# mlysy/rodeo

Hardware: AMD Instinct MI355X
Metric: ODE steps/sec x batch (trajectory-steps/s), FitzHugh-Nagumo q=3, 4000 steps, solve_mv (higher is better)
Workload: dtype f64

## Files before the change

### rodeo_amd/csrc/solve_paths.hpp

```cpp
#pragma once
#include <stdint.h>
#include <stddef.h>
#include <type_traits>
#include <utility>
#include "common.hpp"
#include "rhs.hpp"
#include "solve_args.hpp"

namespace rk {

struct DenseItgArgs;
struct SimLogpost;
struct DaltonObs;

int check_cfg(const rk_solve_cfg* c, const rk_solve_in* in);
int make_args(const rk_solve_cfg* c, const rk_solve_in* in, const rk_solve_out* out, SolveArgs& a);
int begin_solve(rk_handle h);
int small_backward_pass(rk_handle h, const rk_solve_cfg* c, const SolveArgs& a, int mode);

bool dense_supported(const rk_solve_cfg* c, int mode);
int dense_check(const rk_solve_cfg* c, const rk_solve_in* in, int mode);
int dense_solve(rk_handle h, const rk_solve_cfg* c, const rk_solve_in* in, const rk_solve_out* out, int mode);
size_t dense_ws_bytes(const rk_solve_cfg* c, int mode);

enum JitKind : int {
    JIT_FWD = 0,
    JIT_FWD_STORE_PRED = 1,
    JIT_ITG = 2,
    JIT_TILE3 = 3,
    JIT_TILE4 = 4,
    JIT_TILEN = 5,
    JIT_SQRT = 6,
    JIT_FWD_M = 7,
    JIT_FWD_M_STORE_PRED = 8,
    JIT_DENSE_ITG = 9,
    JIT_ITG_M = 10,
    JIT_DALTON = 11,
    JIT_DALTON_STORE = 12,
    JIT_DALTON_TILE3 = 13,
    JIT_DALTON_TILE3_STORE = 14,
};
bool is_user_rhs(int rhs_id);
bool user_tile_available(const rk_solve_cfg* c, JitKind tile);
int user_forward_tile(rk_handle h, const rk_solve_cfg* c, const SolveArgs& a, double* tiles, JitKind tile);
int user_forward(rk_handle h, const rk_solve_cfg* c, const SolveArgs& a);
int user_forward_sqrt(rk_handle h, const rk_solve_cfg* c, const SolveArgs& a);
int user_rhs_check(const rk_solve_cfg* c);
int user_dalton(rk_handle h, const rk_solve_cfg* c, const SolveArgs& a, const DaltonObs& o, int n_bobs, bool store,
                bool tile, double* out);
int user_interrogate(rk_handle h, const rk_solve_cfg* c, const SolveArgs& a, double t, int step, const double* mp,
                     const double* vp, double* wm, double* mm_, double* vm);
bool user_dense_wanted(const rk_solve_cfg* c);
int user_dense_interrogate(rk_handle h, const rk_solve_cfg* c, const DenseItgArgs& a);

int sqrt_solve(rk_handle h, const rk_solve_cfg* c, const SolveArgs& a, int mode, double* ws, size_t ws_bytes);
size_t sqrt_ws_doubles(const rk_solve_cfg* c, int mode);
size_t fenrir_sqrt_item_doubles(int p);
int fenrir_sqrt_launch(rk_handle h, const rk_solve_cfg* c, const SolveArgs& a, const double* obs, const double* obs_w,
                       const double* obs_v, const int32_t* obs_ind, int n_obs, int n_bobs, double* logdens, double* states);

bool tile3_supported(const rk_solve_cfg* c, int mode);
int tile3_solve(rk_handle h, const rk_solve_cfg* c, const SolveArgs& a, double* tiles, int mode, const SimLogpost* lp = nullptr);
int tile3_backward(rk_handle h, const SolveArgs& a, double* tiles, int mode, const SimLogpost* lp = nullptr);
bool tile3_sim_logpost_supported(const rk_solve_cfg* c, int n_obs);
int tile3_solve_sim_logpost(rk_handle h, const rk_solve_cfg* c, const SolveArgs& a, double* tiles, const double* obs,
                            const int32_t* obs_ind, int n_obs, double noise_sd, const double* upars, int n_prior, double prior_sd,
                            double* logpost);
int tile3_fenrir_backward(rk_handle h, const SolveArgs& a, const double* tiles, const double* obs, const double* obs_w,
                          const double* obs_v, const int32_t* obs_ind, int n_obs, double* logdens);
bool tile4_supported(const rk_solve_cfg* c, int mode);
int tile4_solve(rk_handle h, const rk_solve_cfg* c, const SolveArgs& a, double* tiles, int mode);
size_t tile4_doubles(const rk_solve_cfg* c);
bool tilen_supported(const rk_solve_cfg* c, int mode);
int tilen_solve(rk_handle h, const rk_solve_cfg* c, const SolveArgs& a, double* tiles, double* ws, size_t ws_bytes, int mode);
size_t tilen_tile_doubles(const rk_solve_cfg* c);
size_t tilen_ws_doubles(const rk_solve_cfg* c, int mode);

enum class SolvePath { Dense, Sqrt, Tile3, Tile4, TileN, Small };

inline SolvePath solve_path(const rk_solve_cfg* c, int mode) {
    if (dense_supported(c, mode)) return SolvePath::Dense;
    if (tile4_supported(c, mode)) return SolvePath::Tile4;
    if (tile3_supported(c, mode)) return SolvePath::Tile3;
    if (tilen_supported(c, mode)) return SolvePath::TileN;
    return c->kalman_type == RK_KALMAN_SQRT ? SolvePath::Sqrt : SolvePath::Small;
}

inline int path_layout(SolvePath p, const rk_solve_cfg* c) {
    switch (p) {
        case SolvePath::Dense: return RK_LAYOUT_TRAJ_MAJOR;
        case SolvePath::Tile3: return RK_LAYOUT_TILE3;
        case SolvePath::Tile4: return RK_LAYOUT_TILE4;
        case SolvePath::TileN: return c->n_bstate == 4 ? RK_LAYOUT_TILE4 : RK_LAYOUT_TILEP;
        default: return RK_LAYOUT_BATCH_MINOR;
    }
}

template <int Lo, int Hi, class F>
bool dispatch_int(int v, F&& f) {
    if constexpr (Lo > Hi) {
        return false;
    } else {
        if (v == Lo) {
            f(std::integral_constant<int, Lo>{});
            return true;
        }
        return dispatch_int<Lo + 1, Hi>(v, std::forward<F>(f));
    }
}

template <class F>
bool with_builtin_rhs(int rhs_id, F&& f) {
    switch (rhs_id) {
        case RK_RHS_FITZHUGH_NAGUMO: f(FitzHughNagumo{}); return true;
        case RK_RHS_LORENZ63: f(Lorenz63{}); return true;
        case RK_RHS_HIGHER_ORDER: f(HigherOrder{}); return true;
    }
    return false;
}

}
```

### rodeo_amd/csrc/solve_tile3.hip

```cpp
#include <cstdlib>
#include "common.hpp"
#include "kalman_small.hpp"
#include "mfma_tile.hpp"
#include "philox.hpp"
#include "rhs.hpp"
#include "solve_args.hpp"
#include "solve_paths.hpp"
#include "solve_tile3_kernels.hpp"

namespace rk {

constexpr int CHUNK = 16;
constexpr int ITEM_BYTES = 3 * 128;
constexpr int BUF_BYTES = CHUNK * 4 * ITEM_BYTES;
constexpr int ZONE_BYTES = 64 * TILE_DOUBLES * 8;

__device__ __forceinline__ int lds_byte(int s, int g, int which, int idx) {
    const int item = s * 4 + g;
    return item * ITEM_BYTES + which * 128 + (tile_slot(s, g, idx) << 3);
}

__device__ __forceinline__ void tile3_gain_producers(const SolveArgs& a, const double* __restrict__ tiles, int D, int tw, int wave,
                                                     int lane, int n_tiles, size_t tstride, int n_chunks, char* lds_raw,
                                                     char* zones) {
    constexpr int P = 3;
    const int p = wave - 1;
    const int s = lane >> 2, g = lane & 3;
    int tau = tw * 4 + g;
    if (tau >= n_tiles) tau = n_tiles - 1;
    const int b = tau / D, blk = tau - b * D;
    double Q[P][P], R[P][P];
    load_block_consts<P>(a, blk, b, Q, R);
    int woff[12];
#pragma unroll
    for (int i = 0; i < 3; ++i)
#pragma unroll
        for (int j = 0; j < 4; ++j) woff[i * 4 + j] = lds_byte(s, g, 0, i * 4 + j);
    char* const zone = zones + p * ZONE_BYTES;
    const unsigned zone_lds = __builtin_amdgcn_readfirstlane(lds_addr(zone));
    int frow[6], fcol[6];
#pragma unroll
    for (int i = 0; i < 6; ++i) { const int j = 64 * i + lane; frow[i] = j / 24; fcol[i] = (j % 24) * 16; }
    const char* const wave_tiles = (const char*)(tiles + (size_t)tw * 4 * TILE_DOUBLES);
    auto fetch = [&](int ch) {
        const int n_hi = a.N - 1 - ch * CHUNK;
#pragma unroll
        for (int i = 0; i < 6; ++i) {
            const int n = n_hi - frow[i];
            lds_dma16(wave_tiles + (size_t)(n < 1 ? 1 : n) * tstride * 8 + fcol[i], zone_lds + 1024 * i);
        }
    };
    lds_dma_wait_all();
    if (p < n_chunks) fetch(p);
    double mf[P], Sf[P][P], mp[P], Sp[P][P], A[P][P], X[P][P], rpiv[P];
    for (int t = -3; t < n_chunks; ++t) {
        const int ch1 = t + 3, ch2 = t + 2, ch3 = t + 1;
        if (ch1 % 3 == p) {
            if (ch1 < n_chunks) {
                lds_dma_wait_all();
                double buf[TILE_DOUBLES];
#pragma unroll
                for (int k = 0; k < 6; ++k) {
                    const double2 v = *(const double2*)(zone + 96 * lane + 16 * k);
                    buf[2 * k] = v.x; buf[2 * k + 1] = v.y;
                }
                lds_reads_done();
                if (ch1 + 3 < n_chunks) fetch(ch1 + 3);
#pragma unroll
                for (int i = 0; i < P; ++i) {
#pragma unroll
                    for (int j = 0; j < P; ++j) Sf[i][j] = buf[i * 4 + j];
                    mf[i] = buf[i * 4 + 3];
                }
                predict_block<P>(Q, R, mf, Sf, mp, Sp);
            }
        } else if (ch2 >= 0 && ch2 % 3 == p) {
            if (ch2 < n_chunks) {
                double T[P][P];
                mm_nt<P, P, P>(Sf, Q, T);
#pragma unroll
                for (int i = 0; i < P; ++i)
#pragma unroll
                    for (int j = 0; j < P; ++j) { A[i][j] = Sp[i][j]; X[i][j] = T[j][i]; }
                lu_factor_fwd<P, P>(A, X, rpiv);
            }
        } else if (ch3 >= 0) {
            if (ch3 < n_chunks) {
                lu_back<P, P>(A, X, rpiv);
                const int n = a.N - 1 - ch3 * CHUNK - s;
                if (n >= 1) {
                    char* o = lds_raw + (ch3 & 1) * BUF_BYTES;
#pragma unroll
                    for (int i = 0; i < P; ++i) {
#pragma unroll
                        for (int j = 0; j < P; ++j) {
                            *(double*)(o + woff[i * 4 + j]) = Sp[i][j];
                            *(double*)(o + woff[i * 4 + j] + 128) = X[i][j];
                            *(double*)(o + woff[i * 4 + j] + 256) = Sf[i][j];
                        }
                        *(double*)(o + woff[i * 4 + 3]) = mp[i];
                        *(double*)(o + woff[i * 4 + 3] + 256) = mf[i];
                    }
                }
            }
        }
        lds_barrier();   
    }
}

__global__ void __launch_bounds__(256) bwd_mv_tile3_kernel(SolveArgs a, double* __restrict__ tiles, int D) {
    __shared__ __attribute__((aligned(16))) char lds_all[2 * BUF_BYTES];
    __shared__ __attribute__((aligned(16))) char zones[3 * ZONE_BYTES];
    const int wave = threadIdx.x >> 6, lane = threadIdx.x & 63;
    const int n_tiles = a.B * D;
    const size_t tstride = (size_t)n_tiles * TILE_DOUBLES;
    const int n_chunks = (a.N - 1 + CHUNK - 1) / CHUNK;

    for (int i = threadIdx.x; i < 2 * 64 * 3 * 16; i += 256) {
        const int idx = i & 15, which = (i >> 4) % 3, item = ((i >> 4) / 3) & 63, buf = i / (64 * 3 * 16);
        const double v = (idx == 15) ? 1.0 : 0.0;
        *(double*)(lds_all + buf * BUF_BYTES + lds_byte(item >> 2, item & 3, which, idx)) = v;
    }
    __syncthreads();

    const int tw = blockIdx.x;
    char* const lds_raw = lds_all;
    double* const dump = tiles + (size_t)(a.N + 1) * tstride + (size_t)tw * 64;
    const int role = wave;

    if (role >= 1) {
        tile3_gain_producers(a, tiles, D, tw, role, lane, n_tiles, tstride, n_chunks, lds_raw, zones);
    } else {
        const TileCoord tc = tile_coord<1>(tw, lane, n_tiles);
        __builtin_amdgcn_s_setprio(3);
        const int r = tc.r, g = tc.g, c = tc.c, idx = r * 4 + c;
        const bool st = tc.valid && r < 3;
        double* base = st ? tiles + (size_t)tc.tau * TILE_DOUBLES + idx : dump + lane;
        const size_t ostride = st ? tstride : 0;
        int roff[4];
#pragma unroll
        for (int k = 0; k < 4; ++k) roff[k] = lds_byte(k, g, 0, idx) - k * 4 * ITEM_BYTES;
        double Ms = st ? base[(size_t)a.N * ostride] : ((r == 3 && c == 3) ? 1.0 : 0.0);
        const char* const wave_rows = (const char*)(tiles + (size_t)tw * 4 * TILE_DOUBLES);
        const size_t row_bytes = tstride * sizeof(double);
        const unsigned bvoff = st ? (unsigned)((g * TILE_DOUBLES + idx) * sizeof(double)) : 0x80000000u;
        const bool buffer_ok = (CHUNK - 1) * row_bytes + 384 < 0x7fffffffull;
        const int chunk_span = (int)((CHUNK - 1) * row_bytes + 384);
        lds_barrier();
        lds_barrier();
        lds_barrier();
        for (int t = 0; t < n_chunks; ++t) {
            const char* in = lds_raw + (t & 1) * BUF_BYTES;
            const int n_hi = a.N - 1 - t * CHUNK;
            const int cnt = __builtin_amdgcn_readfirstlane(n_hi >= CHUNK ? CHUNK : n_hi);
            double* o = base + (size_t)n_hi * ostride;
            {
                if (cnt == CHUNK && buffer_ok) {
                    constexpr int LOOKAHEAD = 4;
                    double Mp[CHUNK], Gt[CHUNK], Mf[CHUNK];
                    auto load = [&](int s) {
                        const char* q = in + roff[s & 3] + s * 4 * ITEM_BYTES;
                        Mp[s] = *(const double*)(q);
                        Gt[s] = *(const double*)(q + 128);
                        Mf[s] = *(const double*)(q + 256);
                    };
#pragma unroll
                    for (int s = 0; s < LOOKAHEAD; ++s) load(s);
                    const __amdgpu_buffer_rsrc_t rsrc = __builtin_amdgcn_make_buffer_rsrc(
                        (void*)(wave_rows + (size_t)(n_hi - (CHUNK - 1)) * row_bytes), 0, chunk_span, 0x00020000);
                    double Dm = Ms - Mp[0];
#pragma unroll
                    for (int s = 0; s < CHUNK; ++s) {
                        if (s + LOOKAHEAD < CHUNK) load(s + LOOKAHEAD);
                        __builtin_amdgcn_sched_barrier(0);
                        const double V1 = MF(Dm, Gt[s], 0.0);
                        Ms = MF(V1, Gt[s], Mf[s]);
                        if (s + 1 < CHUNK) Dm = Ms - Mp[s + 1];
                        u32x2 bits;
                        __builtin_memcpy(&bits, &Ms, 8);
                        __builtin_amdgcn_raw_buffer_store_b64(bits, rsrc, (int)bvoff, (int)((CHUNK - 1 - s) * row_bytes), 0);
                        __builtin_amdgcn_sched_barrier(0);
                    }
                } else {
                    for (int s = 0; s < cnt; ++s) {
                        const char* q = in + lds_byte(s, g, 0, idx);
                        const double Mp = *(const double*)(q), Gt = *(const double*)(q + 128), Mf = *(const double*)(q + 256);
                        const double V1 = MF(Ms - Mp, Gt, 0.0);
                        Ms = MF(V1, Gt, Mf);
                        o[0] = Ms;
                        o -= ostride;
                    }
                }
            }
            lds_barrier();   
        }
    }
}

struct FenrirObs {
    const double *obs, *obs_w, *obs_v;
    const int32_t* obs_ind;
    int n_obs;
    double* logdens;
};

__global__ void __launch_bounds__(256) fenrir_bwd_tile3_kernel(SolveArgs a, const double* __restrict__ tiles, int D, FenrirObs ob) {
    __shared__ __attribute__((aligned(16))) char lds_all[2 * BUF_BYTES];
    __shared__ __attribute__((aligned(16))) char zones[3 * ZONE_BYTES];
    const int wave = threadIdx.x >> 6, lane = threadIdx.x & 63;
    const int n_tiles = a.B * D;
    const size_t tstride = (size_t)n_tiles * TILE_DOUBLES;
    const int n_chunks = (a.N - 1 + CHUNK - 1) / CHUNK;

    for (int i = threadIdx.x; i < 2 * 64 * 3 * 16; i += 256) {
        const int idx = i & 15, which = (i >> 4) % 3, item = ((i >> 4) / 3) & 63, buf = i / (64 * 3 * 16);
        const double v = (idx == 15) ? 1.0 : 0.0;
        *(double*)(lds_all + buf * BUF_BYTES + lds_byte(item >> 2, item & 3, which, idx)) = v;
    }
    __syncthreads();

    const int tw = blockIdx.x;
    char* const lds_raw = lds_all;

    if (wave >= 1) {
        tile3_gain_producers(a, tiles, D, tw, wave, lane, n_tiles, tstride, n_chunks, lds_raw, zones);
    } else {
        __builtin_amdgcn_s_setprio(3);
        const int r = lane >> 4, g = (lane >> 2) & 3, c = lane & 3, idx = r * 4 + c;
        const int tau_raw = tw * 4 + g;
        const bool valid = tau_raw < n_tiles;
        const int tau = valid ? tau_raw : n_tiles - 1;
        const int b = tau / D, blk = tau - b * D;
        const bool in_tile = valid && r < 3;
        const double e3 = (r == 3 && c == 3) ? 1.0 : 0.0, I4 = r == c ? 1.0 : 0.0;
        const double* const my = tiles + (size_t)tau * TILE_DOUBLES + idx;
        int roff[4];
#pragma unroll
        for (int k = 0; k < 4; ++k) roff[k] = lds_byte(k, g, 0, idx) - k * 4 * ITEM_BYTES;
        double Ms = in_tile ? my[(size_t)a.N * tstride] : e3;
        double acc = 0.0;
        int i = ob.n_obs - 1;
        int next = i >= 0 ? ob.obs_ind[i] : -1;
        auto observe = [&]() {
            const double xw = valid ? (r < 3 ? ob.obs_w[((size_t)i * D + blk) * 3 + r] : -ob.obs[(size_t)i * D + blk]) : 0.0;
            const double Om = valid ? ob.obs_v[(size_t)i * D + blk] : 1.0;
            double MsT = MF(Ms, I4, 0.0);
            MsT = r == 3 ? 0.0 : MsT;
            const double WS = MF(xw, Ms, 0.0);
            const double Z = MF(MsT, xw, 0.0);
            const double w = MF(Z, xw, 0.0) + Om;
            const double z = -quad_bcast3(WS);
            if (fabs(w) > 1e-8) acc += -0.5 * (z * z / w + log(w)) - 0.5 * 1.83787706640934548356;
            const double K = Z / w;
            Ms = fma(-K, WS, Ms);
            --i;
            next = i >= 0 ? ob.obs_ind[i] : -1;
        };
        if (next >= a.N) observe();
        __syncthreads();
        __syncthreads();
        __syncthreads();
        for (int t = 0; t < n_chunks; ++t) {
            const char* in = lds_raw + (t & 1) * BUF_BYTES;
            const int n_hi = a.N - 1 - t * CHUNK;
            const int cnt = __builtin_amdgcn_readfirstlane(n_hi >= CHUNK ? CHUNK : n_hi);
            const bool has_obs = next > n_hi - cnt;
            if (cnt == CHUNK && !has_obs) {
                constexpr int LOOKAHEAD = 4;
                double Mp[CHUNK], Gt[CHUNK], Mf[CHUNK];
                auto load = [&](int s) {
                    const char* q = in + roff[s & 3] + s * 4 * ITEM_BYTES;
                    Mp[s] = *(const double*)(q);
                    Gt[s] = *(const double*)(q + 128);
                    Mf[s] = *(const double*)(q + 256);
                };
#pragma unroll
                for (int s = 0; s < LOOKAHEAD; ++s) load(s);
                double Dm = Ms - Mp[0];
#pragma unroll
                for (int s = 0; s < CHUNK; ++s) {
                    if (s + LOOKAHEAD < CHUNK) load(s + LOOKAHEAD);
                    __builtin_amdgcn_sched_barrier(0);
                    const double V1 = MF(Dm, Gt[s], 0.0);
                    Ms = MF(V1, Gt[s], Mf[s]);
                    if (s + 1 < CHUNK) Dm = Ms - Mp[s + 1];
                    __builtin_amdgcn_sched_barrier(0);
                }
            } else {
                for (int s = 0; s < cnt; ++s) {
                    const char* q = in + lds_byte(s, g, 0, idx);
                    const double Mp = *(const double*)(q), Gt = *(const double*)(q + 128), Mf = *(const double*)(q + 256);
                    const double V1 = MF(Ms - Mp, Gt, 0.0);
                    Ms = MF(V1, Gt, Mf);
                    if (next == n_hi - s) observe();
                }
            }
            __syncthreads();
        }
        if (next == 0) {
            Ms = in_tile ? my[0] : e3;
            observe();
        }
        if (valid && r == 0 && c == 0) atomicAdd(&ob.logdens[b], acc);
    }
}

constexpr int SIM_ITEM = 256;
constexpr int SIM_BUF = CHUNK * 4 * SIM_ITEM;

__device__ __forceinline__ int sim_tile_byte(int s, int g, int idx) {
    const int item = s * 4 + g;
    return item * SIM_ITEM + (tile_slot(s, g, idx) << 3);
}
__device__ __forceinline__ int sim_vec_byte(int s, int g, int which, int rr) {
    const int item = s * 4 + g;
    return item * SIM_ITEM + 128 + (vec_slot(s, g, which, rr) << 3);
}

struct SimLogpost {
    const double* obs;
    const int32_t* obs_ind;
    int n_obs;
    double noise_sd;
    const double* upars;
    int n_prior;
    double prior_sd;
    double* logpost;
};
constexpr int LP_MAX_OBS = 512, LP_MAX_VALS = 1024;

template <bool LP>
__global__ void __launch_bounds__(256, 2) bwd_sim_tile3_kernel(SolveArgs a, double* __restrict__ tiles, int D, SimLogpost lp) {
    constexpr int P = 3;
    __shared__ double lp_obs[LP ? LP_MAX_VALS : 1];
    __shared__ int lp_ind[LP ? LP_MAX_OBS : 1];
    if constexpr (LP) {
        for (int i = threadIdx.x; i < lp.n_obs * D; i += 256) lp_obs[i] = lp.obs[i];
        for (int i = threadIdx.x; i < lp.n_obs; i += 256) { const int ni = lp.obs_ind[i]; lp_ind[i] = ni < 0 ? 0 : (ni > a.N ? a.N : ni); }
    }
    __shared__ __attribute__((aligned(16))) char lds_all[2 * SIM_BUF];
    __shared__ __attribute__((aligned(16))) char zones[3 * ZONE_BYTES];
    constexpr int QR_STRIDE = 2 * 9 + 2;
    __shared__ __attribute__((aligned(16))) double qr[4 * QR_STRIDE];
    const int wave = threadIdx.x >> 6, lane = threadIdx.x & 63;
    const int n_tiles = a.B * D;
    const size_t tstride = (size_t)n_tiles * TILE_DOUBLES;
    const int n_chunks = (a.N + CHUNK - 1) / CHUNK;
// ... 104 lines not shown
                    z[2] = 0.125 + 1e-3 * n; z3 = 0.0;
#else
                    normal_pair(a.seed, traj, (uint32_t)(n < 1 ? 1 : n), (uint32_t)blk, PURPOSE_SMOOTH, 1u, z[2], z3);
#endif
                }
            } else if (ch3 >= 0) {
                if (ch3 < n_chunks) {
                    const int n = a.N - ch3 * CHUNK - s;
                    double GT[P][P], Ssim[P][P], L[P][P], G[P][P];
                    lu_back<P, P>(A, X, rpiv);
                    const bool term = n == a.N;
#pragma unroll
                    for (int i = 0; i < P; ++i)
#pragma unroll
                        for (int j = 0; j < P; ++j) G[i][j] = term ? 0.0 : X[j][i];
                    mm_nt<P, P, P>(G, T, GT);
#pragma unroll
                    for (int i = 0; i < P; ++i)
#pragma unroll
                        for (int j = 0; j < P; ++j) Ssim[i][j] = Sf[i][j] - GT[i][j];
#ifdef RK_T3_ABLATE_SIMPSD
#pragma unroll
                    for (int i = 0; i < P; ++i)
#pragma unroll
                        for (int j = 0; j < P; ++j) L[i][j] = Ssim[i][j];
#else
                    psd_factor<P>(Ssim, L);
#endif
                    if (n >= 1) {
                        char* o = lds_raw + (ch3 & 1) * SIM_BUF;
#pragma unroll
                        for (int i = 0; i < P; ++i) {
                            double w = mf[i];
#pragma unroll
                            for (int k = 0; k <= i; ++k) w = fma(L[i][k], z[k], w);
#pragma unroll
                            for (int j = 0; j < P; ++j) *(double*)(o + woff[i * 3 + j]) = G[j][i];
                            *(double*)(o + voff[i]) = term ? 0.0 : mp[i];
                            *(double*)(o + voff1[i]) = w;
                        }
                    }
                }
            }
            lds_barrier();
        }
    } else {
        const TileCoord tc = tile_coord<1>(tw, lane, n_tiles);
        const int r = tc.r, g = tc.g, c = tc.c, idx = r * 4 + c;
        const int b = tc.tau / D, blk = tc.tau - b * D;
        const bool st = tc.valid && r < 3 && c == 0 && a.x != nullptr;
        const size_t xstride = (size_t)D * P * a.B;
        double* bx = st ? a.x + ((size_t)blk * P + r) * a.B + b : dump + lane;
        const double LOG_SQRT_2PI = 0.91893853320467274178;
        const double lsd = LP ? log(lp.noise_sd) : 0.0;
        int io = LP ? lp.n_obs - 1 : -1;
        double acc = 0.0;
        auto next_index = [&]() { return io >= 0 ? __builtin_amdgcn_readfirstlane(lp_ind[io]) : -1; };
        auto observe = [&](double xv) {
            const double zz = (lp_obs[io * D + blk] - xv) / lp.noise_sd;
            acc += -0.5 * zz * zz - lsd - LOG_SQRT_2PI;
            --io;
        };
        const size_t sx = st ? xstride : 0;
        const bool xbuf_ok = (size_t)CHUNK * xstride * sizeof(double) < 0x7fffffffull;
        const int xvo = st && xbuf_ok ? (int)((((size_t)blk * P + r) * a.B + b) * sizeof(double)) : (int)0x80000000;
        int roff[4], rvec[4], rvec1[4];
#pragma unroll
        for (int k = 0; k < 4; ++k) {
            roff[k] = sim_tile_byte(k, g, idx) - k * 4 * SIM_ITEM;
            rvec[k] = sim_vec_byte(k, g, 0, r) - k * 4 * SIM_ITEM;
            rvec1[k] = sim_vec_byte(k, g, 1, r) - k * 4 * SIM_ITEM;
        }
        double x = 0.0;
        lds_barrier();
        int next_n = LP ? next_index() : -1;
        lds_barrier();
        lds_barrier();
        lds_barrier();
        for (int t = 0; t < n_chunks; ++t) {
            const char* in = lds_raw + (t & 1) * SIM_BUF;
            const int n_hi = a.N - t * CHUNK;
            const int cnt = __builtin_amdgcn_readfirstlane(n_hi >= CHUNK ? CHUNK : n_hi);
            double* o = bx + (size_t)n_hi * sx;
            auto step = [&](const char* q, const char* qv, const char* qw) {
                const double Gt = *(const double*)(q), mp = *(const double*)(qv), mfw = *(const double*)(qw);
                x = MF(Gt, x - mp, mfw);
                o[0] = x;
                o -= sx;
            };
            int n_cur = n_hi;
            if (cnt == CHUNK && xbuf_ok) {
                const __amdgpu_buffer_rsrc_t rsrc = __builtin_amdgcn_make_buffer_rsrc(
                    (void*)(a.x + (size_t)(n_hi - (CHUNK - 1)) * xstride), 0, (int)(CHUNK * xstride * sizeof(double)), 0x00020000);
                double xs[LP ? CHUNK : 1];
#pragma unroll
                for (int s = 0; s < CHUNK; ++s) {
                    const double Gt = *(const double*)(in + roff[s & 3] + s * 4 * SIM_ITEM);
                    const double mp = *(const double*)(in + rvec[s & 3] + s * 4 * SIM_ITEM);
                    const double mfw = *(const double*)(in + rvec1[s & 3] + s * 4 * SIM_ITEM);
                    x = MF(Gt, x - mp, mfw);
                    u32x2 bits;
                    __builtin_memcpy(&bits, &x, 8);
                    __builtin_amdgcn_raw_buffer_store_b64(bits, rsrc, xvo, (int)((CHUNK - 1 - s) * xstride * sizeof(double)), 0);
                    if constexpr (LP) xs[s] = x;
                }
                if constexpr (LP) {
                    if (next_n > n_hi - CHUNK) {
#pragma unroll
                        for (int s = 0; s < CHUNK; ++s)
                            while (n_hi - s == next_n) { observe(xs[s]); next_n = next_index(); }
                    }
                }
            } else if (cnt == CHUNK) {
#pragma unroll
                for (int s = 0; s < CHUNK; ++s) {
                    step(in + roff[s & 3] + s * 4 * SIM_ITEM, in + rvec[s & 3] + s * 4 * SIM_ITEM, in + rvec1[s & 3] + s * 4 * SIM_ITEM);
                    if constexpr (LP) {
                        while (n_cur == next_n) { observe(x); next_n = next_index(); }
                    }
                    --n_cur;
                }
            } else {
                for (int s = 0; s < cnt; ++s) {
                    step(in + sim_tile_byte(s, g, idx), in + sim_vec_byte(s, g, 0, r), in + sim_vec_byte(s, g, 1, r));
                    if constexpr (LP) {
                        while (n_cur == next_n) { observe(x); next_n = next_index(); }
                    }
                    --n_cur;
                }
            }
            lds_barrier();
        }
        const double x_init = tiles[(size_t)tc.tau * TILE_DOUBLES + r * 4 + 3];
        if (st) bx[0] = x_init;
        if constexpr (LP) {
            while (next_n == 0) { observe(x_init); next_n = next_index(); }
            if (D >= 2) acc += __shfl_xor(acc, 4, 64);
            if (D >= 4) acc += __shfl_xor(acc, 8, 64);
            if (tc.valid && r == 0 && c == 0 && blk == 0) {
                if (lp.upars) {
                    const double lps = log(lp.prior_sd);
                    for (int k = 0; k < lp.n_prior; ++k) {
                        const double zz = lp.upars[(size_t)k * a.B + b] / lp.prior_sd;
                        acc += -0.5 * zz * zz - lps - LOG_SQRT_2PI;
                    }
                }
                lp.logpost[b] = acc;
            }
        }
    }
}

template <class RHS>
static int launch_fwd_tile(rk_handle h, const rk_solve_cfg* c, const SolveArgs& a, double* tiles) {
    const dim3 grid(div_up(a.B * RHS::D, Tpw<RHS::D>::value)), block(64);
    launch_placement_primer(h, grid, block);
    LaunchTimer t(h, "fwd_tile3_kernel");
    switch (c->interrogate) {
        case RK_INTERROGATE_KRAMER:
            hipLaunchKernelGGL((fwd_tile3_kernel<RHS, RK_INTERROGATE_KRAMER>), grid, block, 0, h->stream, a, tiles); break;
        case RK_INTERROGATE_SCHOBER:
            hipLaunchKernelGGL((fwd_tile3_kernel<RHS, RK_INTERROGATE_SCHOBER>), grid, block, 0, h->stream, a, tiles); break;
        case RK_INTERROGATE_RODEO:
            hipLaunchKernelGGL((fwd_tile3_kernel<RHS, RK_INTERROGATE_RODEO>), grid, block, 0, h->stream, a, tiles); break;
        case RK_INTERROGATE_CHKREBTII:
            hipLaunchKernelGGL((fwd_tile3_kernel<RHS, RK_INTERROGATE_CHKREBTII>), grid, block, 0, h->stream, a, tiles); break;
        default:
            set_error("tile path: interrogate id %d not supported", c->interrogate);
            return RK_ERR_UNSUPPORTED;
    }
    t.stop();
    RK_HIP(hipGetLastError());
    return RK_OK;
}

bool tile3_supported(const rk_solve_cfg* c, int mode) {
    if (c->flags & (RK_FLAG_STORE_PRED | RK_FLAG_BATCH_MINOR)) return false;
    if (c->kalman_type != RK_KALMAN_STANDARD || c->n_bstate != 3 || c->n_bmeas != 1) return false;
    if (c->interrogate < RK_INTERROGATE_RODEO || c->interrogate > RK_INTERROGATE_CHKREBTII) return false;
    if (c->rhs_id == RK_RHS_FITZHUGH_NAGUMO) return c->n_block == 2;
    if (c->rhs_id == RK_RHS_LORENZ63) return c->n_block == 3;
    if (c->rhs_id == RK_RHS_HIGHER_ORDER) return c->n_block == 1;
    if (is_user_rhs(c->rhs_id)) return user_tile_available(c, JIT_TILE3);
    return false;
}

bool tile3_sim_logpost_supported(const rk_solve_cfg* c, int n_obs) {
    return tile3_supported(c, RK_MODE_SIM) && (c->n_block == 1 || c->n_block == 2 || c->n_block == 4) && n_obs <= LP_MAX_OBS &&
           n_obs * c->n_block <= LP_MAX_VALS;
}

int tile3_solve_sim_logpost(rk_handle h, const rk_solve_cfg* c, const SolveArgs& a, double* tiles, const double* obs,
                            const int32_t* obs_ind, int n_obs, double noise_sd, const double* upars, int n_prior, double prior_sd,
                            double* logpost) {
    SimLogpost lp;
    lp.obs = obs; lp.obs_ind = obs_ind; lp.n_obs = n_obs; lp.noise_sd = noise_sd; lp.upars = upars; lp.n_prior = n_prior;
    lp.prior_sd = prior_sd; lp.logpost = logpost;
    return tile3_solve(h, c, a, tiles, RK_MODE_SIM, &lp);
}

int tile3_solve(rk_handle h, const rk_solve_cfg* c, const SolveArgs& a, double* tiles, int mode, const SimLogpost* lp) {
    int rc = RK_ERR_UNSUPPORTED;
    if (is_user_rhs(c->rhs_id)) rc = user_forward_tile(h, c, a, tiles, JIT_TILE3);
    else with_builtin_rhs(c->rhs_id, [&](auto rhs) { rc = launch_fwd_tile<decltype(rhs)>(h, c, a, tiles); });
    if (rc || mode == RK_MODE_FILTER) return rc;
    return tile3_backward(h, a, tiles, mode, lp);
}

int tile3_backward(rk_handle h, const SolveArgs& a, double* tiles, int mode, const SimLogpost* lp) {
    if (mode == RK_MODE_SIM) {
        LaunchTimer t(h, "bwd_sim_tile3_kernel");
        if (lp) hipLaunchKernelGGL(bwd_sim_tile3_kernel<true>, dim3(div_up(a.B * a.D, 4)), dim3(256), 0, h->stream, a, tiles, a.D, *lp);
        else hipLaunchKernelGGL(bwd_sim_tile3_kernel<false>, dim3(div_up(a.B * a.D, 4)), dim3(256), 0, h->stream, a, tiles, a.D, SimLogpost{});
        t.stop();
        RK_HIP(hipGetLastError());
        return RK_OK;
    }
    if (a.N < 2) return RK_OK;
    LaunchTimer t(h, "bwd_mv_tile3_kernel");
    hipLaunchKernelGGL(bwd_mv_tile3_kernel, dim3(div_up(a.B * a.D, 4)), dim3(256), 0, h->stream, a, tiles, a.D);
    t.stop();
    RK_HIP(hipGetLastError());
    return RK_OK;
}

int tile3_fenrir_backward(rk_handle h, const SolveArgs& a, const double* tiles, const double* obs, const double* obs_w,
                          const double* obs_v, const int32_t* obs_ind, int n_obs, double* logdens) {
    FenrirObs ob;
    ob.obs = obs; ob.obs_w = obs_w; ob.obs_v = obs_v; ob.obs_ind = obs_ind; ob.n_obs = n_obs; ob.logdens = logdens;
    LaunchTimer t(h, "fenrir_bwd_tile3_kernel");
    hipLaunchKernelGGL(fenrir_bwd_tile3_kernel, dim3(div_up(a.B * a.D, 4)), dim3(256), 0, h->stream, a, tiles, a.D, ob);
    t.stop();
    RK_HIP(hipGetLastError());
    return RK_OK;
}

}
```

### rodeo_amd/csrc/solve_tile3_kernels.hpp

```cpp
#pragma once
#include "rk_enums.hpp"
#include "kalman_small.hpp"
#include "mfma_tile.hpp"
#include "philox.hpp"
#include "solve_args.hpp"

namespace rk {

constexpr int TILE_DOUBLES = 12;
typedef unsigned int u32x2 __attribute__((ext_vector_type(2)));

struct TileCoord {
    int r, g, c;
    int tau;
    int b, blk;
    bool valid;
};

template <int D, int TPW = 4>
__device__ __forceinline__ TileCoord tile_coord(int wave, int lane, int n_tiles) {
    TileCoord t;
    t.r = lane >> 4; t.g = (lane >> 2) & 3; t.c = lane & 3;
    const int tau = wave * TPW + t.g;
    t.valid = t.g < TPW && tau < n_tiles;
    t.tau = t.valid ? tau : (wave * TPW < n_tiles ? wave * TPW : n_tiles - 1);
    t.b = t.tau / D; t.blk = t.tau - t.b * D;
    return t;
}

constexpr int TILE_MAX_BLOCKS = 64;

template <int D>
struct TileWaves {
    static constexpr int value = D <= 4 ? 1 : (D + 3) / 4;
};

__device__ __forceinline__ double sqrt_pos_1step(double x) {
    const double rs = __builtin_amdgcn_rsq(x);
    const double g = x * rs, h = 0.5 * rs;
    const double s = fma(fma(-g, g, x), h, g);
    return x > 0.0 ? s : 0.0;
}

template <class RHS, int ITG>
__global__ void __launch_bounds__(64 * TileWaves<RHS::D>::value) fwd_tile3_kernel(SolveArgs a, double* __restrict__ tiles) {
    constexpr int D = RHS::D, P = 3, NW = TileWaves<D>::value, TPW = NW > 1 ? 4 : Tpw<D>::value;
    static_assert(D >= 1 && D <= TILE_MAX_BLOCKS, "tile path: n_block in 1..64");
    static_assert(RHS::NDEP == 1, "tile path: right-hand sides that depend on X[b][0] only");
    const int n_tiles = a.B * D;
    const int wave_in_wg = threadIdx.x >> 6, lane = threadIdx.x & 63;
    TileCoord tc;
    if constexpr (NW == 1) {
        tc = tile_coord<D, TPW>(blockIdx.x, lane, n_tiles);
    } else {
        tc.r = lane >> 4; tc.g = (lane >> 2) & 3; tc.c = lane & 3;
        const int blk_w = wave_in_wg * 4 + tc.g;
        tc.valid = blk_w < D;
        tc.b = blockIdx.x; tc.blk = tc.valid ? blk_w : D - 1;
        tc.tau = tc.b * D + tc.blk;
    }
    const int r = tc.r, c = tc.c, b = tc.b, blk = tc.blk;
    const bool in3 = r < 3 && c < 3;

    const double Qt = in3 ? ld(a.Q, ((size_t)blk * P + c) * P + r, a.Q_b, a.B, b) : ((r == 3 && c == 3) ? 1.0 : 0.0);
    const double Qt0 = in3 ? Qt : 0.0;
    const double Rt = in3 ? ld(a.R, ((size_t)blk * P + r) * P + c, a.R_b, a.B, b) : 0.0;
    const double RtT = in3 ? ld(a.R, ((size_t)blk * P + c) * P + r, a.R_b, a.B, b) : 0.0;
    const double Wr = r < 3 ? ld(a.W, (size_t)blk * P + r, a.W_b, a.B, b) : 0.0;
    const double Y0 = r < 3 ? ld(a.Q, ((size_t)blk * P + 0) * P + r, a.Q_b, a.B, b) : 0.0;
    const double E0 = r == 0 ? 1.0 : 0.0;
    const double e3r = r == 3 ? 1.0 : 0.0;
    double th[RHS::NTHETA];
#pragma unroll
    for (int k = 0; k < RHS::NTHETA; ++k) th[k] = a.theta ? ld(a.theta, k, a.theta_b, a.B, b) : 0.0;
    double c3 = 0.0, c2 = 0.0, c1 = 0.0, co = 0.0, c0 = Wr;
    if constexpr (rhs_has_tile_form<RHS>::value && D == 2) {
        double tk[6];
        RHS::tile_consts(blk, th, tk);
        const bool jac = ITG == RK_INTERROGATE_KRAMER;
        const double k4 = jac ? tk[4] : 0.0, k5 = jac ? tk[5] : 0.0;
        if (r == 3) { c3 = k5 - tk[1]; c1 = k4 - tk[0]; co = -tk[2]; c0 = -tk[3]; }
        if (r == 0) { c2 = -k5; c0 = Wr - k4; }
    }
    __shared__ double zbuf_all[NW][4 * 16];
    double* const zbuf = zbuf_all[wave_in_wg];
    __shared__ double vx[2][NW > 1 ? TILE_MAX_BLOCKS : 1];
    const uint32_t traj = (uint32_t)(a.traj_offset + (uint64_t)b);

    double M = r < 3 ? (c == 3 ? ld(a.x0, (size_t)blk * P + r, a.x0_b, a.B, b) : 0.0) : (c == 3 ? 1.0 : 0.0);
    const bool st = tc.valid && r < 3;
    const size_t tstride_all = (size_t)n_tiles * TILE_DOUBLES;
    const char* row = (const char*)(tiles + (NW == 1 ? (size_t)blockIdx.x * TPW : (size_t)blockIdx.x * D + (size_t)wave_in_wg * 4) * TILE_DOUBLES);
    const int bvoff = st ? (int)((tc.g * TILE_DOUBLES + r * 4 + c) * sizeof(double)) : (int)0x80000000;
    auto store_row = [&](double v) {
        const __amdgpu_buffer_rsrc_t rsrc = __builtin_amdgcn_make_buffer_rsrc((void*)row, 0, TPW * TILE_DOUBLES * 8, 0x00020000);
        u32x2 bits;
        __builtin_memcpy(&bits, &v, 8);
        __builtin_amdgcn_raw_buffer_store_b64(bits, rsrc, bvoff, 0, 0);
    };
#define RK_STORE_BEHIND(M_, mfma_result)                              \
    do {                                                              \
        asm("" : "+v"(M_) : "v"(mfma_result));                        \
        store_row(M_);                                                \
        row += tstride_all * sizeof(double);                          \
    } while (0)

    if constexpr (rhs_has_tile_form<RHS>::value && D == 2 && ITG != RK_INTERROGATE_CHKREBTII) {
#define RK_AFTER(in, res) asm("" : "+v"(in) : "v"(res))
        for (int n = 0; n < a.N; ++n) {
            double U = MF(M, Qt, 0.0);
            RK_STORE_BEHIND(M, U);
            double B0 = MF(Y0, M, 0.0);
            RK_AFTER(U, B0);
            double MpT = MF(Qt0, U, RtT);
            RK_AFTER(B0, MpT);
            const double v_own = quad_bcast3(B0);
            const double v_oth = pair_other_quad_uniform(v_own);
            const double Xw = fma(fma(fma(c3, v_own, c2), v_own, c1), v_own, fma(co, v_oth, c0));
            RK_AFTER(U, Xw);
            double Mp = MF(U, Qt, Rt);
            RK_AFTER(MpT, Mp);
            double Z0 = MF(MpT, Xw, 0.0);
            RK_AFTER(Mp, Z0);
            double WS = MF(Xw, Mp, 0.0);
            RK_AFTER(Z0, WS);
            double S = MF(Z0, Xw, 0.0);
            RK_AFTER(WS, S);
            if constexpr (ITG == RK_INTERROGATE_RODEO) S = S + S;
            const double PW = Z0 * WS;
            RK_AFTER(S, PW);
            const double y0 = __builtin_amdgcn_rcp(S);
            const double e = fma(-S, y0, 1.0);
            const double y = fma(y0, fma(e, e, e), y0);
            M = fma(-PW, y, Mp);
        }
        store_row(M);
#undef RK_AFTER
#ifdef RK_PLACEMENT_DEBUG
        if (lane == 0) {
            double* tail = tiles + (size_t)(a.N + 1) * tstride_all + (size_t)blockIdx.x * 64;
            tail[0] = (double)__builtin_amdgcn_s_getreg((31 << 11) | 4);
            tail[1] = (double)__builtin_amdgcn_s_getreg((31 << 11) | 20);
        }
#endif
        return;
    }
    if constexpr (rhs_has_tile_form<RHS>::value && D == 2 && ITG == RK_INTERROGATE_CHKREBTII) {
        double tk[6];
        RHS::tile_consts(blk, th, tk);
        const double ac3 = -tk[1], ac1 = -tk[0], aco = -tk[2], ac0 = -tk[3];
        const double e3c = c == 3 ? 1.0 : 0.0;
        for (int n = 0; n < a.N; ++n) {
#if defined(RK_T3_ABLATE) && RK_T3_ABLATE >= 1
            const double zn = 0.25;
#else
            if ((n & 15) == 0) {
                double z0, z1;
                normal_pair(a.seed, traj, (uint32_t)(n + r * 4 + c), (uint32_t)blk, PURPOSE_INTERROGATE, 0u, z0, z1);
                zbuf[tc.g * 16 + r * 4 + c] = z0;
            }
            const double zn = zbuf[tc.g * 16 + (n & 15)];
#endif
            const double U = MF(M, Qt, 0.0);
            RK_STORE_BEHIND(M, U);
            const double Mp = MF(U, Qt, Rt);
            const double MpT = MF(Qt0, U, RtT);
            const double R0 = MF(E0, Mp, 0.0);
            double Z0 = MF(MpT, Wr, 0.0);
            const double WS0 = MF(Wr, Mp, 0.0);
            asm("" : "+v"(Z0) : "v"(WS0));
            double S = MF(Z0, Wr, 0.0);
            S = S + S;
            const double rS = fast_rcp_cubic(S);
            double r0v = R0;
            asm("" : "+v"(r0v) : "v"(rS));
#if defined(RK_T3_ABLATE) && RK_T3_ABLATE >= 2
            const double v_own = fma(quad_bcast0(r0v), zn, quad_bcast3(r0v));
#else
            const double v_own = fma(sqrt_pos_1step(quad_bcast0(r0v)), zn, quad_bcast3(r0v));
#endif
            const double v_oth = pair_other_quad_uniform(v_own);
            const double am = fma(fma(fma(ac3, v_own, 0.0), v_own, ac1), v_own, fma(aco, v_oth, ac0));
            const double WS = fma(e3c, am, WS0);
            const double PW = Z0 * WS;
            M = fma(-PW, rS, Mp);
        }
        store_row(M);
        return;
    }
    double l0 = 0.0, l1 = 0.0, l2 = 0.0, l3 = 0.0, l4 = 0.0, XwL = 0.0;
    if constexpr (rhs_has_tile3_form<RHS>::value && D == 3 && NW == 1) {
        double kk[5];
        RHS::tile3_consts(blk, th, kk);
        const bool jac = ITG == RK_INTERROGATE_KRAMER;
        l0 = jac ? 0.0 : -kk[0]; l1 = -kk[1]; l2 = -kk[2]; l3 = -kk[3]; l4 = -kk[4];
        XwL = fma(jac ? -kk[0] : 0.0, E0, Wr);
    }
    for (int n = 0; n < a.N; ++n) {
        const double U = MF(M, Qt, 0.0);
        RK_STORE_BEHIND(M, U);
        double v_own;
        if constexpr (ITG != RK_INTERROGATE_CHKREBTII) v_own = quad_bcast3(MF(Y0, M, 0.0));
        const double Mp = MF(U, Qt, Rt);
        const double MpT = MF(Qt0, U, RtT);
        if constexpr (ITG == RK_INTERROGATE_CHKREBTII) {
            if ((n & 15) == 0) {
                double z0, z1;
                normal_pair(a.seed, traj, (uint32_t)(n + r * 4 + c), (uint32_t)blk, PURPOSE_INTERROGATE, 0u, z0, z1);
                zbuf[tc.g * 16 + r * 4 + c] = z0;
            }
            const double zn = zbuf[tc.g * 16 + (n & 15)];
            const double R0 = MF(E0, Mp, 0.0);
            const double s00 = quad_bcast0(R0);
            v_own = fma(sqrt(s00 > 0.0 ? s00 : 0.0), zn, quad_bcast3(R0));
        }
        const double t = a.t_min + (a.t_max - a.t_min) * (double)(n + 1) / (double)a.N;
        double Xw;
        if constexpr (rhs_has_tile_form<RHS>::value && D == 2) {
            const double v_oth = pair_other_quad_uniform(v_own);
            Xw = fma(fma(fma(c3, v_own, c2), v_own, c1), v_own, fma(co, v_oth, c0));
        } else if constexpr (rhs_has_tile3_form<RHS>::value && D == 3 && NW == 1) {
            const double n1 = from_next_tile(v_own), p1 = from_prev_tile(v_own), p2 = dpp64<0x128>(v_own);
            const double a_meas = fma(l4, p2 * p1, fma(l3, p1 * n1, fma(l2, p1, fma(l1, n1, l0 * v_own))));
            Xw = fma(a_meas, e3r, XwL);
        } else {
            constexpr int PX = 1;
            double X[D][PX];
            if constexpr (NW == 1) {
                double vals[D];
                gather_blocks<D>(v_own, vals);
#pragma unroll
                for (int bb = 0; bb < D; ++bb) X[bb][0] = vals[bb];
            } else {
                if (tc.valid && r == 0 && c == 0) vx[n & 1][blk] = v_own;
                __syncthreads();
#pragma unroll
                for (int bb = 0; bb < D; ++bb) X[bb][0] = vx[n & 1][bb];
            }
            double fb, J0;
            if constexpr (ITG == RK_INTERROGATE_KRAMER && rhs_has_fjac0<RHS>::value) {
                RHS::template fjac0_block<PX>(X, t, th, blk, fb, J0);
            } else if constexpr (ITG != RK_INTERROGATE_KRAMER && rhs_has_f_block<RHS>::value) {
                fb = RHS::template f_block<PX>(X, t, th, blk);
                J0 = 0.0;
            } else {
                double f[D], J[D][PX];
                if constexpr (ITG == RK_INTERROGATE_KRAMER) {
                    RHS::template fjac<PX>(X, t, th, f, J);
                } else {
                    RHS::template f<PX>(X, t, th, f);
#pragma unroll
                    for (int bb = 0; bb < D; ++bb)
#pragma unroll
                        for (int j = 0; j < PX; ++j) J[bb][j] = 0.0;
                }
                double J0s[D];
#pragma unroll
                for (int bb = 0; bb < D; ++bb) J0s[bb] = J[bb][0];
                fb = pick_block<D>(f, blk); J0 = pick_block<D>(J0s, blk);
            }
            const double a_meas = fma(J0, v_own, -fb);
            Xw = fma(-J0, E0, fma(a_meas, e3r, Wr));
        }
        const double WS = MF(Xw, Mp, 0.0);
        const double Z0 = MF(MpT, Xw, 0.0);
        double S = MF(Z0, Xw, 0.0);
        if constexpr (ITG == RK_INTERROGATE_RODEO || ITG == RK_INTERROGATE_CHKREBTII)
            S = S + S;
        const double K = Z0 * fast_rcp_cubic(S);
        M = fma(-K, WS, Mp);
    }
    store_row(M);
#undef RK_STORE_BEHIND
}

}
```

Before: 5.832 billion.

## Pack forward-pass tile records as symmetric 9-double entries to cut traffic

For the FitzHugh-Nagumo two-block mean/variance path, the forward tile kernel now stores only the upper triangle of the 3x3 covariance plus the mean (9 doubles instead of a 16-double tile) per step. It packs four steps into three rows of storage. The backward kernel's gain producers fetch and unpack these compact records, then rebuild the symmetric matrix, and the first-row base value is restored from x0. This is meant to cut global memory write and read bandwidth between the forward and backward passes, at the cost of more complex address arithmetic, a 4x-unrolled forward loop, and an env var to fall back.

```diff
diff --git a/rodeo_amd/csrc/solve_paths.hpp b/rodeo_amd/csrc/solve_paths.hpp
--- a/rodeo_amd/csrc/solve_paths.hpp
+++ b/rodeo_amd/csrc/solve_paths.hpp
@@ -61,7 +61,8 @@
 
 bool tile3_supported(const rk_solve_cfg* c, int mode);
 int tile3_solve(rk_handle h, const rk_solve_cfg* c, const SolveArgs& a, double* tiles, int mode, const SimLogpost* lp = nullptr);
-int tile3_backward(rk_handle h, const SolveArgs& a, double* tiles, int mode, const SimLogpost* lp = nullptr);
+int tile3_backward(rk_handle h, const SolveArgs& a, double* tiles, int mode, const SimLogpost* lp = nullptr,
+                   bool packed = false);
 bool tile3_sim_logpost_supported(const rk_solve_cfg* c, int n_obs);
 int tile3_solve_sim_logpost(rk_handle h, const rk_solve_cfg* c, const SolveArgs& a, double* tiles, const double* obs,
                             const int32_t* obs_ind, int n_obs, double noise_sd, const double* upars, int n_prior, double prior_sd,
diff --git a/rodeo_amd/csrc/solve_tile3.hip b/rodeo_amd/csrc/solve_tile3.hip
--- a/rodeo_amd/csrc/solve_tile3.hip
+++ b/rodeo_amd/csrc/solve_tile3.hip
@@ -20,6 +20,7 @@
     return item * ITEM_BYTES + which * 128 + (tile_slot(s, g, idx) << 3);
 }
 
+template <bool PACKED = false>
 __device__ __forceinline__ void tile3_gain_producers(const SolveArgs& a, const double* __restrict__ tiles, int D, int tw, int wave,
                                                      int lane, int n_tiles, size_t tstride, int n_chunks, char* lds_raw,
                                                      char* zones) {
@@ -42,12 +43,27 @@
 #pragma unroll
     for (int i = 0; i < 6; ++i) { const int j = 64 * i + lane; frow[i] = j / 24; fcol[i] = (j % 24) * 16; }
     const char* const wave_tiles = (const char*)(tiles + (size_t)tw * 4 * TILE_DOUBLES);
+    const int k = n_tiles - tw * 4 < 4 ? n_tiles - tw * 4 : 4, rec = 72 * k, slice = 96 * k;
     auto fetch = [&](int ch) {
         const int n_hi = a.N - 1 - ch * CHUNK;
-#pragma unroll
-        for (int i = 0; i < 6; ++i) {
-            const int n = n_hi - frow[i];
-            lds_dma16(wave_tiles + (size_t)(n < 1 ? 1 : n) * tstride * 8 + fcol[i], zone_lds + 1024 * i);
+        if constexpr (PACKED) {
+            const int n_lo = n_hi - (CHUNK - 1);
+#pragma unroll
+            for (int i = 0; i < 5; ++i) {
+                const int j = 64 * i + lane, jr = 16 * j / rec;
+                if (j < rec) {
+                    int m = n_lo + jr;
+                    m = m < 1 ? 1 : m;
+                    const int o = rec * (m & 3) + 16 * j - jr * rec, rr = o / slice;
+                    lds_dma16(wave_tiles + ((size_t)3 * (m >> 2) + rr) * tstride * 8 + (o - rr * slice), zone_lds + 1024 * i);
+                }
+            }
+        } else {
+#pragma unroll
+            for (int i = 0; i < 6; ++i) {
+                const int n = n_hi - frow[i];
+                lds_dma16(wave_tiles + (size_t)(n < 1 ? 1 : n) * tstride * 8 + fcol[i], zone_lds + 1024 * i);
+            }
         }
     };
     lds_dma_wait_all();
@@ -58,19 +74,32 @@
         if (ch1 % 3 == p) {
             if (ch1 < n_chunks) {
                 lds_dma_wait_all();
-                double buf[TILE_DOUBLES];
-#pragma unroll
-                for (int k = 0; k < 6; ++k) {
-                    const double2 v = *(const double2*)(zone + 96 * lane + 16 * k);
-                    buf[2 * k] = v.x; buf[2 * k + 1] = v.y;
-                }
-                lds_reads_done();
-                if (ch1 + 3 < n_chunks) fetch(ch1 + 3);
-#pragma unroll
-                for (int i = 0; i < P; ++i) {
-#pragma unroll
-                    for (int j = 0; j < P; ++j) Sf[i][j] = buf[i * 4 + j];
-                    mf[i] = buf[i * 4 + 3];
+                if constexpr (PACKED) {
+                    const double* v = (const double*)(zone + rec * (CHUNK - 1 - s) + 72 * (g < k ? g : k - 1));
+                    double buf[9];
+#pragma unroll
+                    for (int e = 0; e < 9; ++e) buf[e] = v[e];
+                    lds_reads_done();
+                    if (ch1 + 3 < n_chunks) fetch(ch1 + 3);
+                    Sf[0][0] = buf[0]; Sf[0][1] = buf[1]; Sf[0][2] = buf[2]; mf[0] = buf[3];
+                    Sf[1][1] = buf[4]; Sf[1][2] = buf[5]; mf[1] = buf[6];
+                    Sf[2][2] = buf[7]; mf[2] = buf[8];
+                    Sf[1][0] = Sf[0][1]; Sf[2][0] = Sf[0][2]; Sf[2][1] = Sf[1][2];
+                } else {
+                    double buf[TILE_DOUBLES];
+#pragma unroll
+                    for (int k = 0; k < 6; ++k) {
+                        const double2 v = *(const double2*)(zone + 96 * lane + 16 * k);
+                        buf[2 * k] = v.x; buf[2 * k + 1] = v.y;
+                    }
+                    lds_reads_done();
+                    if (ch1 + 3 < n_chunks) fetch(ch1 + 3);
+#pragma unroll
+                    for (int i = 0; i < P; ++i) {
+#pragma unroll
+                        for (int j = 0; j < P; ++j) Sf[i][j] = buf[i * 4 + j];
+                        mf[i] = buf[i * 4 + 3];
+                    }
                 }
                 predict_block<P>(Q, R, mf, Sf, mp, Sp);
             }
@@ -108,6 +137,7 @@
     }
 }
 
+template <bool PACKED>
 __global__ void __launch_bounds__(256) bwd_mv_tile3_kernel(SolveArgs a, double* __restrict__ tiles, int D) {
     __shared__ __attribute__((aligned(16))) char lds_all[2 * BUF_BYTES];
     __shared__ __attribute__((aligned(16))) char zones[3 * ZONE_BYTES];
@@ -129,7 +159,7 @@
     const int role = wave;
 
     if (role >= 1) {
-        tile3_gain_producers(a, tiles, D, tw, role, lane, n_tiles, tstride, n_chunks, lds_raw, zones);
+        tile3_gain_producers<PACKED>(a, tiles, D, tw, role, lane, n_tiles, tstride, n_chunks, lds_raw, zones);
     } else {
         const TileCoord tc = tile_coord<1>(tw, lane, n_tiles);
         __builtin_amdgcn_s_setprio(3);
@@ -193,6 +223,12 @@
                 }
             }
             lds_barrier();   
+        }
+        if constexpr (PACKED) {
+            if (st) {
+                const int b = tc.tau / D, blk = tc.tau - b * D;
+                base[0] = c == 3 ? ld(a.x0, (size_t)blk * 3 + r, a.x0_b, a.B, b) : 0.0;
+            }
         }
     }
 }
@@ -603,10 +639,28 @@
 }
 
 template <class RHS>
-static int launch_fwd_tile(rk_handle h, const rk_solve_cfg* c, const SolveArgs& a, double* tiles) {
+static int launch_fwd_tile(rk_handle h, const rk_solve_cfg* c, const SolveArgs& a, double* tiles, bool packed) {
     const dim3 grid(div_up(a.B * RHS::D, Tpw<RHS::D>::value)), block(64);
     launch_placement_primer(h, grid, block);
     LaunchTimer t(h, "fwd_tile3_kernel");
+    if constexpr (rhs_has_tile_form<RHS>::value && RHS::D == 2) {
+        if (packed) {
+            switch (c->interrogate) {
+                case RK_INTERROGATE_KRAMER:
+                    hipLaunchKernelGGL((fwd_tile3_kernel<RHS, RK_INTERROGATE_KRAMER, true>), grid, block, 0, h->stream, a, tiles); break;
+                case RK_INTERROGATE_SCHOBER:
+                    hipLaunchKernelGGL((fwd_tile3_kernel<RHS, RK_INTERROGATE_SCHOBER, true>), grid, block, 0, h->stream, a, tiles); break;
+                case RK_INTERROGATE_RODEO:
+                    hipLaunchKernelGGL((fwd_tile3_kernel<RHS, RK_INTERROGATE_RODEO, true>), grid, block, 0, h->stream, a, tiles); break;
+                default:
+                    set_error("tile path: packed records with interrogate id %d", c->interrogate);
+                    return RK_ERR_UNSUPPORTED;
+            }
+            t.stop();
+            RK_HIP(hipGetLastError());
+            return RK_OK;
+        }
+    }
     switch (c->interrogate) {
         case RK_INTERROGATE_KRAMER:
             hipLaunchKernelGGL((fwd_tile3_kernel<RHS, RK_INTERROGATE_KRAMER>), grid, block, 0, h->stream, a, tiles); break;
@@ -650,15 +704,24 @@
     return tile3_solve(h, c, a, tiles, RK_MODE_SIM, &lp);
 }
 
+static bool tile3_packed_records(const rk_solve_cfg* c, const SolveArgs& a, int mode) {
+    if (mode != RK_MODE_MV || c->rhs_id != RK_RHS_FITZHUGH_NAGUMO || c->n_block != 2 || c->interrogate == RK_INTERROGATE_CHKREBTII)
+        return false;
+    if (a.N < 2 || 2 * (size_t)a.B * a.D * TILE_DOUBLES * sizeof(double) + 384 >= 0x7fffffffull) return false;
+    const char* e = getenv("RK_TILE3_FULL_RECORDS");
+    return !(e && atoi(e) != 0);
+}
+
 int tile3_solve(rk_handle h, const rk_solve_cfg* c, const SolveArgs& a, double* tiles, int mode, const SimLogpost* lp) {
     int rc = RK_ERR_UNSUPPORTED;
+    const bool packed = tile3_packed_records(c, a, mode);
     if (is_user_rhs(c->rhs_id)) rc = user_forward_tile(h, c, a, tiles, JIT_TILE3);
-    else with_builtin_rhs(c->rhs_id, [&](auto rhs) { rc = launch_fwd_tile<decltype(rhs)>(h, c, a, tiles); });
+    else with_builtin_rhs(c->rhs_id, [&](auto rhs) { rc = launch_fwd_tile<decltype(rhs)>(h, c, a, tiles, packed); });
     if (rc || mode == RK_MODE_FILTER) return rc;
-    return tile3_backward(h, a, tiles, mode, lp);
-}
-
-int tile3_backward(rk_handle h, const SolveArgs& a, double* tiles, int mode, const SimLogpost* lp) {
+    return tile3_backward(h, a, tiles, mode, lp, packed);
+}
+
+int tile3_backward(rk_handle h, const SolveArgs& a, double* tiles, int mode, const SimLogpost* lp, bool packed) {
     if (mode == RK_MODE_SIM) {
         LaunchTimer t(h, "bwd_sim_tile3_kernel");
         if (lp) hipLaunchKernelGGL(bwd_sim_tile3_kernel<true>, dim3(div_up(a.B * a.D, 4)), dim3(256), 0, h->stream, a, tiles, a.D, *lp);
@@ -669,7 +732,8 @@
     }
     if (a.N < 2) return RK_OK;
     LaunchTimer t(h, "bwd_mv_tile3_kernel");
-    hipLaunchKernelGGL(bwd_mv_tile3_kernel, dim3(div_up(a.B * a.D, 4)), dim3(256), 0, h->stream, a, tiles, a.D);
+    if (packed) hipLaunchKernelGGL(bwd_mv_tile3_kernel<true>, dim3(div_up(a.B * a.D, 4)), dim3(256), 0, h->stream, a, tiles, a.D);
+    else hipLaunchKernelGGL(bwd_mv_tile3_kernel<false>, dim3(div_up(a.B * a.D, 4)), dim3(256), 0, h->stream, a, tiles, a.D);
     t.stop();
     RK_HIP(hipGetLastError());
     return RK_OK;
diff --git a/rodeo_amd/csrc/solve_tile3_kernels.hpp b/rodeo_amd/csrc/solve_tile3_kernels.hpp
--- a/rodeo_amd/csrc/solve_tile3_kernels.hpp
+++ b/rodeo_amd/csrc/solve_tile3_kernels.hpp
@@ -42,11 +42,13 @@
     return x > 0.0 ? s : 0.0;
 }
 
-template <class RHS, int ITG>
+template <class RHS, int ITG, bool PACKED = false>
 __global__ void __launch_bounds__(64 * TileWaves<RHS::D>::value) fwd_tile3_kernel(SolveArgs a, double* __restrict__ tiles) {
     constexpr int D = RHS::D, P = 3, NW = TileWaves<D>::value, TPW = NW > 1 ? 4 : Tpw<D>::value;
     static_assert(D >= 1 && D <= TILE_MAX_BLOCKS, "tile path: n_block in 1..64");
     static_assert(RHS::NDEP == 1, "tile path: right-hand sides that depend on X[b][0] only");
+    static_assert(!PACKED || (rhs_has_tile_form<RHS>::value && D == 2 && ITG != RK_INTERROGATE_CHKREBTII),
+                  "packed records: the headline step only");
     const int n_tiles = a.B * D;
     const int wave_in_wg = threadIdx.x >> 6, lane = threadIdx.x & 63;
     TileCoord tc;
@@ -107,33 +109,93 @@
 
     if constexpr (rhs_has_tile_form<RHS>::value && D == 2 && ITG != RK_INTERROGATE_CHKREBTII) {
 #define RK_AFTER(in, res) asm("" : "+v"(in) : "v"(res))
-        for (int n = 0; n < a.N; ++n) {
-            double U = MF(M, Qt, 0.0);
-            RK_STORE_BEHIND(M, U);
-            double B0 = MF(Y0, M, 0.0);
-            RK_AFTER(U, B0);
-            double MpT = MF(Qt0, U, RtT);
-            RK_AFTER(B0, MpT);
-            const double v_own = quad_bcast3(B0);
-            const double v_oth = pair_other_quad_uniform(v_own);
-            const double Xw = fma(fma(fma(c3, v_own, c2), v_own, c1), v_own, fma(co, v_oth, c0));
-            RK_AFTER(U, Xw);
-            double Mp = MF(U, Qt, Rt);
-            RK_AFTER(MpT, Mp);
-            double Z0 = MF(MpT, Xw, 0.0);
-            RK_AFTER(Mp, Z0);
-            double WS = MF(Xw, Mp, 0.0);
-            RK_AFTER(Z0, WS);
-            double S = MF(Z0, Xw, 0.0);
-            RK_AFTER(WS, S);
-            if constexpr (ITG == RK_INTERROGATE_RODEO) S = S + S;
-            const double PW = Z0 * WS;
-            RK_AFTER(S, PW);
-            const double y0 = __builtin_amdgcn_rcp(S);
-            const double e = fma(-S, y0, 1.0);
-            const double y = fma(y0, fma(e, e, e), y0);
-            M = fma(-PW, y, Mp);
-        }
+        if constexpr (PACKED) {
+            const char* prow = row;
+            const int row_bytes = (int)(tstride_all * sizeof(double));
+            int pspan, pv[4];
+            {
+                const int k = n_tiles - (int)blockIdx.x * TPW < TPW ? n_tiles - (int)blockIdx.x * TPW : TPW;
+                const int kap = r * 4 - r * (r + 1) / 2 + c;
+                const bool slot = st && c >= r;
+#pragma unroll
+                for (int ph = 0; ph < 4; ++ph) {
+                    const int o = 72 * k * ph + 72 * tc.g + 8 * kap, rr = o / (96 * k);
+                    pv[ph] = slot ? rr * row_bytes + (o - rr * 96 * k) : (int)0x80000000;
+                }
+                pspan = 2 * row_bytes + 96 * k;
+            }
+            auto store_packed = [&](double v, int voff) {
+                const __amdgpu_buffer_rsrc_t rsrc = __builtin_amdgcn_make_buffer_rsrc((void*)prow, 0, pspan, 0x00020000);
+                u32x2 bits;
+                __builtin_memcpy(&bits, &v, 8);
+                __builtin_amdgcn_raw_buffer_store_b64(bits, rsrc, voff, 0, 0);
+            };
+            auto step = [&](int voff) __attribute__((always_inline)) {
+                double U = MF(M, Qt, 0.0);
+                asm("" : "+v"(M) : "v"(U));
+                store_packed(M, voff);
+                double B0 = MF(Y0, M, 0.0);
+                RK_AFTER(U, B0);
+                double MpT = MF(Qt0, U, RtT);
+                RK_AFTER(B0, MpT);
+                const double v_own = quad_bcast3(B0);
+                const double v_oth = pair_other_quad_uniform(v_own);
+                const double Xw = fma(fma(fma(c3, v_own, c2), v_own, c1), v_own, fma(co, v_oth, c0));
+                RK_AFTER(U, Xw);
+                double Mp = MF(U, Qt, Rt);
+                RK_AFTER(MpT, Mp);
+                double Z0 = MF(MpT, Xw, 0.0);
+                RK_AFTER(Mp, Z0);
+                double WS = MF(Xw, Mp, 0.0);
+                RK_AFTER(Z0, WS);
+                double S = MF(Z0, Xw, 0.0);
+                RK_AFTER(WS, S);
+                if constexpr (ITG == RK_INTERROGATE_RODEO) S = S + S;
+                const double PW = Z0 * WS;
+                RK_AFTER(S, PW);
+                const double y0 = __builtin_amdgcn_rcp(S);
+                const double e = fma(-S, y0, 1.0);
+                const double y = fma(y0, fma(e, e, e), y0);
+                M = fma(-PW, y, Mp);
+            };
+            int n = 0;
+            for (; n + 4 <= a.N; n += 4) {
+                step(pv[0]); step(pv[1]); step(pv[2]); step(pv[3]);
+                prow += 3 * (size_t)row_bytes;
+            }
+            if (n < a.N) step(pv[0]);
+            if (n + 1 < a.N) step(pv[1]);
+            if (n + 2 < a.N) step(pv[2]);
+            row += (size_t)a.N * row_bytes;
+        } else {
+            for (int n = 0; n < a.N; ++n) {
+                double U = MF(M, Qt, 0.0);
+                RK_STORE_BEHIND(M, U);
+                double B0 = MF(Y0, M, 0.0);
+                RK_AFTER(U, B0);
+                double MpT = MF(Qt0, U, RtT);
+                RK_AFTER(B0, MpT);
+                const double v_own = quad_bcast3(B0);
+                const double v_oth = pair_other_quad_uniform(v_own);
+                const double Xw = fma(fma(fma(c3, v_own, c2), v_own, c1), v_own, fma(co, v_oth, c0));
+                RK_AFTER(U, Xw);
+                double Mp = MF(U, Qt, Rt);
+                RK_AFTER(MpT, Mp);
+                double Z0 = MF(MpT, Xw, 0.0);
+                RK_AFTER(Mp, Z0);
+                double WS = MF(Xw, Mp, 0.0);
+                RK_AFTER(Z0, WS);
+                double S = MF(Z0, Xw, 0.0);
+                RK_AFTER(WS, S);
+                if constexpr (ITG == RK_INTERROGATE_RODEO) S = S + S;
+                const double PW = Z0 * WS;
+                RK_AFTER(S, PW);
+                const double y0 = __builtin_amdgcn_rcp(S);
+                const double e = fma(-S, y0, 1.0);
+                const double y = fma(y0, fma(e, e, e), y0);
+                M = fma(-PW, y, Mp);
+            }
+            }
         store_row(M);
 #undef RK_AFTER
 #ifdef RK_PLACEMENT_DEBUG
```

After: 5.908 billion, median of 6. 1.01x the previous value.
